# ChangwuLiu/InGVIO

Hardware: AMD Instinct MI355X
Metric: ekf_updates_per_sec (higher is better)
Workload: dtype f64; 1 GPU; BASELINE configs[1]: synthetic stereo MSCKF, 150 feats x 11 clones, state dim N=249 (update at N), 512 independent filters per GPU; step = propagate(k=10)+clone+MSCKF update+marginalise; filters_per_gpu=512, feats=150, clones=11, state_dim=249, imu_steps=10, parallelism=independent filters, 1 rank(s), no data-path collective

## Files before the change

include/ingvio_hip.h:

```cpp
#ifndef INGVIO_HIP_H
#define INGVIO_HIP_H

#include <stddef.h>

#ifdef __cplusplus
extern "C" {
#endif

#define INGVIO_OK 0
#define INGVIO_NO_ROWS 1
#define INGVIO_NEG_DIAG 2
#define INGVIO_REJECTED 3
#define INGVIO_E_ARG (-1)
#define INGVIO_E_CAPACITY (-2)
#define INGVIO_E_HIP (-3)
#define INGVIO_E_NOT_IN_STATE (-4)
#define INGVIO_E_UNSUPPORTED (-5)
#define INGVIO_E_NOT_PD (-6)

typedef struct ingvio_ctx ingvio_ctx;

typedef struct {
    int batch;
    int n_max;
// ... 323 lines not shown
    double psr_noise_amp, dopp_noise_amp;
} ingvio_gnss_epoch_nominal;
int ingvio_gnss_front_stage_nominal(ingvio_ctx* ctx, int b0, int nb, const ingvio_gnss_epoch_nominal* epochs, const ingvio_gnss_opts* opts);
int ingvio_gnss_frame_stage_nominal(ingvio_ctx* ctx, int b0, int nb, const ingvio_gnss_epoch_nominal* epochs, const ingvio_gnss_opts* opts);
int ingvio_debug_gnss_fused_last(ingvio_ctx* ctx);
int ingvio_debug_nominal_update_post(ingvio_ctx* ctx, int b0, int nb, const double* dx, const int* marg_idx);
typedef struct {
    int n_lm;
    const int* lm_var;
    const double* uv;
    const unsigned char* tracked;
} ingvio_landmark_frame_nominal;
int ingvio_landmark_stage_nominal(ingvio_ctx* ctx, int b0, int nb, const ingvio_landmark_frame_nominal* frames,
                                  const ingvio_landmark_opts* opts);
typedef struct {
    int track;
    int anchor;
    double pf[3];
} ingvio_lm_init_cand;
typedef struct {
    int n_cand; const ingvio_lm_init_cand* cand;
    int n_drop; const int* drop_cols;
} ingvio_lm_init_block;
int ingvio_landmark_init_nominal(ingvio_ctx* ctx, int b0, int nb, const ingvio_lm_init_block* blocks, const ingvio_msckf_opts* opts,
                                 double chi2_mult, int do_chi2, int cand_cap,
                                 int* added, int* new_idx, int* slot, double* chi2, double* dx, int* status);
int ingvio_debug_landmark_init_rows(ingvio_ctx* ctx, int b, const ingvio_lm_init_cand* cand, const ingvio_msckf_opts* opts,
                                    int n_drop, const int* drop_cols, double* H_old, double* H_new, double* res, int* m_out);
int ingvio_frame_run(ingvio_ctx* ctx, int restore_prior);
int ingvio_set_frame_parts(ingvio_ctx* ctx, int parts);
int ingvio_set_gram_reduced(ingvio_ctx* ctx, int on);
int ingvio_set_gram_decoupled(ingvio_ctx* ctx, int on);
int ingvio_last_gram_form(ingvio_ctx* ctx);
int ingvio_set_delayed_form(ingvio_ctx* ctx, int mode);
int ingvio_frame_fetch(ingvio_ctx* ctx, int b0, int nb, double* dx_out, int* accepted, int* rows_out);
int ingvio_frame_fetch_begin(ingvio_ctx* ctx, int b0, int nb);
int ingvio_frame_fetch_end(ingvio_ctx* ctx, double* dx_out, int* accepted, int* rows_out);

int ingvio_debug_msckf_info(ingvio_ctx* ctx, int b, double* A_out, int* ncol_out);

int ingvio_debug_info_solution(ingvio_ctx* ctx, int b, double* out, int count);

int ingvio_debug_tracks_read(ingvio_ctx* ctx, int b, unsigned long long* mask, double* uv, double* pf);

int ingvio_debug_staged_frame(ingvio_ctx* ctx, int b, int* n_clones, int* n_feat, int* clone_idx, double* clone_R, double* clone_p,
                              int* anchor, int* dof, unsigned long long* obs_mask, double* pf, double* uv);

int ingvio_debug_read(ingvio_ctx* ctx, long long* out, int n);

int ingvio_profile_enable(ingvio_ctx* ctx, int enable);
int ingvio_profile_select(ingvio_ctx* ctx, const char* kernel_name);
int ingvio_profile_reset(ingvio_ctx* ctx);
int ingvio_profile_get(ingvio_ctx* ctx, const char** names, double* ms, int* calls, int cap);

#ifdef __cplusplus
}
#endif
#endif
```

ingvio_amd/capi.py:

```python
import ctypes as C
import os

import numpy as np

_HERE = os.path.dirname(os.path.abspath(__file__))
LIB_PATH = os.environ.get("INGVIO_HIP_LIB") or os.path.join(_HERE, "lib", "libingvio_hip.so")

c_dp = C.POINTER(C.c_double)
c_ip = C.POINTER(C.c_int)
c_up = C.POINTER(C.c_ulonglong)

OK, NO_ROWS, NEG_DIAG, REJECTED = 0, 1, 2, 3
E_ARG, E_CAPACITY, E_HIP, E_NOT_IN_STATE, E_UNSUPPORTED, E_NOT_PD = -1, -2, -3, -4, -5, -6
R_SCALAR, R_DIAG, R_FULL = 0, 1, 2

EXPORTS = [
    "ingvio_ctx_create", "ingvio_ctx_destroy", "ingvio_sync", "ingvio_ctx_stream", "ingvio_f_max", "ingvio_c_max", "ingvio_last_error", "ingvio_ldp",
    "ingvio_build_id",
    "ingvio_cov_set", "ingvio_cov_get", "ingvio_get_n", "ingvio_cov_get_marginal", "ingvio_cov_snapshot",
    "ingvio_cov_restore", "ingvio_propagate", "ingvio_propagate_fused", "ingvio_augment_clone", "ingvio_marginalize",
    "ingvio_append_independent", "ingvio_ekf_update", "ingvio_chi2_gamma", "ingvio_msckf_update", "ingvio_msckf_update_tri", "ingvio_qr_compress",
    "ingvio_frame_stage", "ingvio_frame_stage_async", "ingvio_frame_set_imu_noise", "ingvio_frame_fetch_begin", "ingvio_frame_fetch_end", "ingvio_tracks_create", "ingvio_frame_stage_tracks", "ingvio_frame_run", "ingvio_set_frame_parts", "ingvio_set_gram_reduced", "ingvio_set_gram_decoupled", "ingvio_last_gram_form", "ingvio_frame_fetch", "ingvio_profile_enable", "ingvio_profile_select",
    "ingvio_profile_reset",
    "ingvio_profile_get", "ingvio_set_msckf_method", "ingvio_set_qr_method", "ingvio_landmark_stage", "ingvio_landmark_run",
    "ingvio_landmark_fetch", "ingvio_frame_run_phase", "ingvio_info_set", "ingvio_debug_read", "ingvio_triangulate",
    "ingvio_gnss_front_stage", "ingvio_gnss_front_fetch", "ingvio_gnss_update_batch", "ingvio_gnss_stage", "ingvio_gnss_run", "ingvio_gnss_fetch", "ingvio_mld", "ingvio_debug_msckf_info", "ingvio_debug_info_solution",
    "ingvio_info_reduce", "ingvio_info_commit", "ingvio_gnss_sat_eval",
    "ingvio_chi2_gamma_multi", "ingvio_ekf_update_batch", "ingvio_add_variable_delayed_invertible", "ingvio_add_variable_delayed", "ingvio_add_variable_delayed_batch", "ingvio_replace_var_linear",
    "ingvio_nominal_create", "ingvio_nominal_set", "ingvio_nominal_get", "ingvio_nominal_box_plus", "ingvio_frame_stage_tracks_nominal",
    "ingvio_nominal_set_gnss", "ingvio_nominal_get_gnss", "ingvio_gnss_front_stage_nominal", "ingvio_landmark_stage_nominal",
    "ingvio_landmark_init_nominal", "ingvio_debug_landmark_init_rows", "ingvio_nominal_tail",
    "ingvio_debug_tracks_read", "ingvio_debug_staged_frame",
    "ingvio_gnss_frame_stage_nominal", "ingvio_debug_gnss_fused_last", "ingvio_debug_nominal_update_post",
    "ingvio_update_stage_tracks_nominal", "ingvio_frame_fetch_tri", "ingvio_set_delayed_form",
    "ingvio_odom_begin", "ingvio_odom_end", "ingvio_cov_get_marginal_batch",
    "ingvio_frame_stage_tracks_nominal_tri", "ingvio_set_first_tri_placement",
]

NOM_NONE, NOM_SE23, NOM_SE3, NOM_VEC3, NOM_SCALAR, NOM_LANDMARK = -1, 0, 1, 2, 3, 4
NOM_VAL = 15
ODOM_COV, ODOM_EUCL, ODOM_DIAG = 1, 2, 4
ODOM_ALL = ODOM_COV | ODOM_EUCL | ODOM_DIAG
ODOM_NONFINITE, ODOM_NEG_DIAG, ODOM_ABSENT = 1, 2, 4
MARGINAL_NS_MAX = 64


class GateBlock(C.Structure):
    _fields_ = [("vidx", C.POINTER(C.c_int)), ("vsize", C.POINTER(C.c_int)), ("k", C.c_int), ("H", C.POINTER(C.c_double)),
                ("ldh", C.c_int), ("m", C.c_int), ("res", C.POINTER(C.c_double))]


class UpdateBlock(C.Structure):
    _fields_ = [("vidx", C.POINTER(C.c_int)), ("vsize", C.POINTER(C.c_int)), ("k", C.c_int), ("H", C.POINTER(C.c_double)),
                ("ldh", C.c_int), ("m", C.c_int), ("res", C.POINTER(C.c_double)), ("R", C.POINTER(C.c_double))]

# ... 1022 lines not shown
        nb = len(steps)
        sa = (FrameStep * nb)(); fa = (MsckfFrame * nb)()
        keeps = []
        for i in range(nb):
            s, k1 = make_step(steps[i]); f, k2 = make_frame(frames[i])
            sa[i] = s; fa[i] = f; keeps.append((k1, k2))
        o, chi2 = make_opts(frames[0], max_accept, compress_rule, selected_variant)
        sg = f64(sigma)

        fn = self.L.ingvio_frame_stage_async if use_async else self.L.ingvio_frame_stage

        def call(_keep=(keeps, chi2, sa, fa, o, sg)):
            self._chk(fn(self.h, b0, nb, sa, fa, C.byref(o), _d(sg), int(enable_gnss), C.c_double(sigma_cb), C.c_double(sigma_rw)))
        return call

    def frame_set_imu_noise(self, b0, noise):
        nz = f64(np.asarray(noise, dtype=np.float64).reshape(-1, 6))
        self._chk(self.L.ingvio_frame_set_imu_noise(self.h, int(b0), nz.shape[0], _d(nz)))

    def frame_run(self, restore_prior=False):
        self._chk(self.L.ingvio_frame_run(self.h, 1 if restore_prior else 0))

    def set_frame_parts(self, parts):
        self._chk(self.L.ingvio_set_frame_parts(self.h, int(parts)))

    def set_gram_reduced(self, on):
        self._chk(self.L.ingvio_set_gram_reduced(self.h, 1 if on else 0))

    def set_gram_decoupled(self, on):
        self._chk(self.L.ingvio_set_gram_decoupled(self.h, 1 if on else 0))

    def last_gram_form(self):
        return int(self.L.ingvio_last_gram_form(self.h))

    def set_delayed_form(self, mode):
        self._chk(self.L.ingvio_set_delayed_form(self.h, int(mode)))

    def frame_fetch(self, b0=0, nb=None):
        nb = self.batch if nb is None else nb
        dx = np.zeros((nb, self.ldp)); acc = np.zeros((nb, self.f_max), dtype=np.int32); rows = np.zeros(nb, dtype=np.int32)
        self._chk(self.L.ingvio_frame_fetch(self.h, b0, nb, _d(dx), _i(acc), _i(rows)))
        return dx, acc, rows

    def frame_fetch_begin(self, b0=0, nb=None):
        nb = self.batch if nb is None else nb
        self._fetch_nb = nb
        self._chk(self.L.ingvio_frame_fetch_begin(self.h, b0, nb))

    def frame_fetch_end(self):
        nb = self._fetch_nb
        dx = np.empty((nb, self.ldp)); acc = np.empty((nb, self.f_max), dtype=np.int32); rows = np.empty(nb, dtype=np.int32)
        self._chk(self.L.ingvio_frame_fetch_end(self.h, _d(dx), _i(acc), _i(rows)))
        return dx, acc, rows

    def triangulate(self, b0, frames, stereo=True, mask_failed=False, **params):
        pr = dict(trans_thres=0.1, huber_epsilon=0.01, conv_precision=5e-7, init_damping=1e-3, outer_loop_max_iter=10,
                  inner_loop_max_iter=10, max_depth=60.0, min_depth=0.2)
        pr.update(params)
        o = TriOpts()
        o.stereo = 1 if stereo else 0
        ref = frames[0] if frames else None
        Rl = f64(ref["R_cl2cr"]).reshape(-1) if ref is not None else np.eye(3).reshape(-1)
        tl = f64(ref["t_cl2cr"]) if ref is not None else np.zeros(3)
        if "R_cl2cr" in params:
            Rl = f64(pr.pop("R_cl2cr")).reshape(-1)
        if "t_cl2cr" in params:
# ... 83 lines not shown
```

ingvio_amd/csrc/capi.hip:

```cpp
#include "../../include/ingvio_hip.h"
#include "dev_common.h"
#include "launch_ekf.h"
#include "launch_msckf.h"
#include "launch_factored.h"
#include "launch_tri.h"
#include "launch_tracks.h"
#include "launch_lm.h"
#include "launch_delayed.h"
#include "launch_qr.h"
#include "launch_chol.h"
#include "launch_gnss.h"
#include "launch_lmbatch.h"
#include "launch_nominal.h"
#include "launch_tail.h"
#include "launch_odom.h"

#include <stdio.h>
#include <stdlib.h>
#include <string.h>
#include <unistd.h>
#include <string>
#include <atomic>
#include <cmath>
#include <condition_variable>
// ... 115 lines not shown
    MsckfOpts st_op;
    std::vector<int> st_gnss;
    std::vector<int> st_marg;
    std::vector<int> st_cidx_hi;
    bool staged;
    double* d_xchg = nullptr;
    bool phase_pending = false;
    struct InputSet {
        double *Phi = nullptr, *G = nullptr, *dt = nullptr, *R = nullptr, *clone_R = nullptr, *clone_p = nullptr, *pf = nullptr, *uv = nullptr,
               *chi2 = nullptr, *noise = nullptr, *prm = nullptr;
        int *gnss = nullptr, *idx = nullptr, *clone_idx = nullptr, *nclones = nullptr, *nfeat = nullptr, *anchor = nullptr, *dof = nullptr;
        unsigned long long* mask = nullptr;
    } alt;
    bool alt_ready = false;
    hipStream_t st2 = nullptr;
    hipEvent_t ev_fork = nullptr, ev_join = nullptr, ev_ref = nullptr;
    hipEvent_t ev_fetch = nullptr;
    int fetch_b0 = 0, fetch_nb = 0;
    hipStream_t st_copy = nullptr;
    hipEvent_t ev_copy = nullptr, ev_free[2] = { nullptr, nullptr };
    bool copy_pending = false, free_valid[2] = { false, false };
    int set_id = 0;
    struct PinSlab { char* p = nullptr; size_t cap = 0; hipEvent_t ev = nullptr; bool busy = false; };
    PinSlab pin[4];
    int pin_next = 0;
    struct PartStream { hipStream_t st = nullptr; hipEvent_t ev_gate = nullptr, ev_apply = nullptr, ev_done = nullptr; };
    PartStream part[4];
    int parts_alloc = 0;
    int parts_req = -1;
    int gram_reduced = 1;
    int delayed_form = 0;
    int gram_decoupled = 1;
    int gram_form_last = 0;
    int gram_red_last = 0;
    bool split_pending = false;
    hipEvent_t tok_last = nullptr;
    hipEvent_t ev_split_fork = nullptr;
    hipStream_t run_st = nullptr;
    hipEvent_t tok_wait = nullptr, tok_rec = nullptr;
    struct Tracks { double *uv = nullptr, *pf = nullptr; unsigned long long* mask = nullptr; int t_max = 0; char* stage[2] = { nullptr, nullptr }; size_t stage_cap = 0; } trk;
    struct Nominal {
        int vmax = 0, ir = 0, dr = 0;
        int* ih = nullptr; double* dv = nullptr;
        int* ih_snap = nullptr; double* dv_snap = nullptr;
        double* dx = nullptr;
        std::vector<int> h_ih, h_ih_snap;
        bool has_snap = false;
        bool pending = false;
        bool frame = false;
        hipEvent_t ev = nullptr; bool ev_valid = false;
        bool noprop = false, tri_on = false, tri_ran = false;
        int tri_fmx = 0;
        bool tri_fetched = false; int tri_b0 = 0, tri_nb = 0;
        ingvio_tri_opts tri;
        int* d_tri_track = nullptr;
        int tri_place = 0;
        bool tri_staged = false;
        int* d_tri_ok_st = nullptr; double* d_tri_pf_st = nullptr;
    } nom;
    struct TailWs { char *in = nullptr, *ws = nullptr, *h_out = nullptr; size_t in_cap = 0, ws_cap = 0, out_cap = 0; } tl;
    struct OdomOut {
        double *d = nullptr, *h = nullptr; hipEvent_t ev = nullptr; bool pending = false; int b0 = 0, nb = 0;
        int *cols = nullptr, *ns = nullptr; double* blk = nullptr; size_t cols_cap = 0, blk_cap = 0;
    } od;
    bool prof;
    std::vector<ProfRec> recs;
// ... 606 lines not shown
                if (used) c->recs.push_back({ PF_GATE2, L.prof_a, L.prof_b });
                else { hipEventDestroy(L.prof_a); hipEventDestroy(L.prof_b); }
                L.prof_a = nullptr; L.prof_b = nullptr; L.prof_used = nullptr;
            }
            if (grc) return INGVIO_E_UNSUPPORTED;
        }
        c->gram_red_last = 0; c->gram_form_last = 0;
        L.gram_red = frame_step && phase == 0 && c->gram_reduced; L.gram_was_red = &c->gram_red_last;
        L.gram_dec = c->gram_decoupled; L.gram_form = &c->gram_form_last;
        { ProfScope p(c, PF_GRAM); L.stage = 1; launch_factored(L, c->run_st); }
        L.gram_was_red = nullptr; L.gram_form = nullptr;
        if (c->tok_rec) HIPCHK(c, hipEventRecord(c->tok_rec, c->run_st));
    }
    if (forked) {
        HIPCHK(c, hipStreamWaitEvent(c->st2, c->ev_fork, 0));
        L.stage = 6; launch_factored(L, c->st2);
        HIPCHK(c, hipEventRecord(c->ev_ref, c->st2));
        L.stage = 7; launch_factored(L, c->st2);
        HIPCHK(c, hipEventRecord(c->ev_join, c->st2));
    }
    if (phase == 1) return last_launch(c);
    if (forked) {
        ProfScope p(c, PF_INFO);
        HIPCHK(c, hipStreamWaitEvent(c->run_st, c->ev_ref, 0));
        L.stage = 8; launch_factored(L, c->run_st);
        HIPCHK(c, hipStreamWaitEvent(c->run_st, c->ev_join, 0));
        L.stage = 9; launch_factored(L, c->run_st);
    } else {
        if (big) { ProfScope p(c, PF_INFO); L.stage = 5; launch_factored(L, c->run_st); }
        { ProfScope p(c, PF_INFO); L.stage = 2; launch_factored(L, c->run_st); }
    }
    if (gnss_fuse) { if (int rc = gnss_in_frame_launch(c, b0, nb, L)) return rc; }
    if (phase == 2 && c->tok_wait) HIPCHK(c, hipStreamWaitEvent(c->run_st, c->tok_wait, 0));
    { ProfScope p(c, PF_APPLY); L.stage = 3; launch_factored(L, c->run_st); }
    if (phase == 2 && c->tok_rec) HIPCHK(c, hipEventRecord(c->tok_rec, c->run_st));
    return last_launch(c);
}

int run_msckf(ingvio_ctx* c, int b0, int nb, const MsckfOpts& op, int stereo, int fmax_used)
{
    if (c->method == 1) return run_msckf_factored(c, b0, nb, op, stereo, fmax_used);
    c->gram_red_last = 0; c->gram_form_last = 0;
    MsckfLaunch L;
    memset(&L, 0, sizeof L);
    L.stereo = stereo; L.cv = view(c); L.fv = fview(c); L.op = op; L.b0 = b0; L.nb = nb;
    L.fmax_used = fmax_used > 0 ? fmax_used : 1;
    L.gamma = c->d_gamma; L.accept = c->d_accept; L.used = c->d_used;
    L.Rpart = c->d_Rpart + (size_t)b0 * c->G * c->rstride; L.chunk_used = c->d_chunk_used + (size_t)b0 * c->G;
    L.G = c->G; L.rstride = c->rstride;
    L.Hout = c->d_H + (size_t)b0 * c->hstride; L.res_out = c->d_res + (size_t)b0 * c->mld;
    L.colmap = c->d_colmap + (size_t)b0 * c->cstride; L.m_out = c->d_m + b0; L.nc_out = c->d_nc + b0;
    L.mld = c->mld; L.hstride = c->hstride; L.cstride = c->cstride;
    { ProfScope p(c, PF_GATE); L.stage = 0; if (launch_msckf(L, c->st)) return INGVIO_E_UNSUPPORTED; }
    { ProfScope p(c, PF_FOLD); L.stage = 1; launch_msckf(L, c->st); }
    { ProfScope p(c, PF_MERGE); L.stage = 2; launch_msckf(L, c->st); }
    EkfLaunch E;
    memset(&E, 0, sizeof E);
    E.cv = view(c); E.b0 = b0; E.nb = nb; E.H = L.Hout; E.res = L.res_out; E.colmap = L.colmap; E.m = L.m_out; E.nc = L.nc_out;
    E.noise = c->d_noise + b0; E.r_kind = 0; E.mld = c->mld; E.hstride = c->hstride; E.cstride = c->cstride; E.nstride = 1;
    E.Y = c->d_Y + (size_t)b0 * c->ystride; E.ystride = c->ystride; E.dx = c->d_dx; E.status = c->d_status;
    E.m_cap = 6 * c->d.c_max; E.nc_cap = 6 * c->d.c_max;
    { ProfScope p(c, PF_EKF_CORE); launch_ekf_core(E, c->st); }
    { ProfScope p(c, PF_DOWNDATE); launch_downdate(E, c->d.n_max, c->st); }
    return last_launch(c);
}

// ... 111 lines not shown
        c->nom.frame = plan != nullptr;
        c->nom.noprop = upd; c->nom.tri_on = false; c->nom.tri_staged = false;
        c->st_stereo = opts->stereo; c->st_enable_gnss = enable_gnss;
        if (!c->staged || fmx > c->st_fmax_used) c->st_fmax_used = fmx;
        c->staged = true;
        return INGVIO_OK;
    }
};

}

extern "C" {

int ingvio_ctx_create(const ingvio_ctx_desc* desc, ingvio_ctx** out)
{
    if (!desc || !out || desc->batch < 1 || desc->n_max < 21 || desc->c_max < 1 || desc->f_max < 1) return INGVIO_E_ARG;
    if (desc->c_max > bigwin_cmax()) return INGVIO_E_CAPACITY;
    if (desc->m_max > 128) return INGVIO_E_CAPACITY;
    int ndev = 0;
    if (hipGetDeviceCount(&ndev) != hipSuccess || ndev <= desc->device) return INGVIO_E_HIP;
    ingvio_ctx* c = new ingvio_ctx();
    c->d = *desc;
    if (c->d.m_max < 1) c->d.m_max = 32;
    c->err.clear();
    if (hipSetDevice(desc->device) != hipSuccess) { delete c; return INGVIO_E_HIP; }
    c->own_stream = desc->stream == nullptr;
    if (c->own_stream) {
        if (hipStreamCreateWithFlags(&c->st, hipStreamNonBlocking) != hipSuccess) { delete c; return INGVIO_E_HIP; }
    } else c->st = (hipStream_t)desc->stream;
    c->run_st = c->st;
    if (const char* e = getenv("INGVIO_FRAME_PARTS")) c->parts_req = atoi(e);
    if (const char* e = getenv("INGVIO_GRAM_REDUCED")) c->gram_reduced = atoi(e) != 0;
    if (const char* e = getenv("INGVIO_GRAM_DECOUPLED")) c->gram_decoupled = atoi(e) != 0;
    if (desc->c_max > 16) {
        int lo = 0, hi = 0;
        hipDeviceGetStreamPriorityRange(&lo, &hi);
        if (hipStreamCreateWithPriority(&c->st2, hipStreamNonBlocking, hi) != hipSuccess) c->st2 = nullptr;
        if (c->st2 && (hipEventCreateWithFlags(&c->ev_fork, hipEventDisableTiming) != hipSuccess ||
                       hipEventCreateWithFlags(&c->ev_ref, hipEventDisableTiming) != hipSuccess ||
                       hipEventCreateWithFlags(&c->ev_join, hipEventDisableTiming) != hipSuccess)) { hipStreamDestroy(c->st2); c->st2 = nullptr; }
    }
    const int B = desc->batch;
    c->ldp = (desc->n_max + 15) & ~15;
    const int cls0 = desc->c_max > 16 ? bigwin_cmax() : msckf_cmax_class(desc->c_max);
    const int cpad = cls0 > desc->c_max ? cls0 : desc->c_max;
    const int mcap = c->d.m_max > 6 * cpad ? c->d.m_max : 6 * cpad;
    c->mld = (mcap + 15) & ~15;
    c->nc_cap = c->ldp > mcap ? c->ldp : mcap;
    c->G = (desc->c_max > 16 ? 256 : 512) / B;
    { const int gmax = desc->c_max > 16 ? 32 : 16; if (c->G > gmax) c->G = gmax; }
    if (c->G < 1) c->G = 1;
#ifdef INGVIO_ALT_KERNELS
    if (const char* e = getenv("INGVIO_GRAM_CHUNKS")) { const int g = atoi(e); if (g >= 1 && g <= 64) c->G = g; }
#endif
    c->cls = msckf_cmax_class(desc->c_max);
    const int ncm = 6 * desc->c_max;
    c->rstride = ncm * (ncm + 1);
    c->hstride = c->mld * c->nc_cap;
    c->cstride = c->nc_cap;
    c->ystride = std::max(c->ldp * (c->mld + 4), c->mld * (c->mld + 1));
    c->has_snap = false; c->staged = false; c->prof = false;
    c->method = 1;
#ifdef INGVIO_ALT_KERNELS
    if (const char* e = getenv("INGVIO_MSCKF_METHOD")) c->method = (!strcmp(e, "dense") || !strcmp(e, "0")) ? 0 : 1;
#endif
    memset(c->prof_ms, 0, sizeof c->prof_ms); memset(c->prof_calls, 0, sizeof c->prof_calls);
// ... 3264 lines not shown
    const bool gnss_fuse = gnss_folds(c);
    if (P > 1 && c->method == 1 && !lm_in_frame(c) && c->d.c_max <= 16 && (!gnss_in_frame(c) || gnss_fuse) && B >= 16 * P)
        return frame_run_split(c, restore_prior, P, gnss_fuse);
    return frame_run_whole(c, restore_prior);
}

int ingvio_frame_run(ingvio_ctx* c, int restore_prior) { return frame_run_impl(c, restore_prior, 0); }
int ingvio_set_frame_parts(ingvio_ctx* c, int parts)
{
    if (!c || parts < -1 || parts > 4) return INGVIO_E_ARG;
    ENTER(c);
    c->parts_req = parts == 0 ? 1 : parts;
    return INGVIO_OK;
}
int ingvio_set_gram_reduced(ingvio_ctx* c, int on)
{
    if (!c) return INGVIO_E_ARG;
    ENTER(c);
    c->gram_reduced = on ? 1 : 0;
    return INGVIO_OK;
}
int ingvio_set_gram_decoupled(ingvio_ctx* c, int on)
{
    if (!c) return INGVIO_E_ARG;
    ENTER(c);
    c->gram_decoupled = on ? 1 : 0;
    return INGVIO_OK;
}
int ingvio_last_gram_form(ingvio_ctx* c)
{
    if (!c) return INGVIO_E_ARG;
    return c->gram_form_last;
}
int ingvio_set_delayed_form(ingvio_ctx* c, int mode)
{
    if (!c) return INGVIO_E_ARG;
    ENTER(c);
    if (mode < 0 || mode > 2) { c->err = "ingvio_set_delayed_form: mode is 0, 1 or 2"; return INGVIO_E_ARG; }
    if (phase_busy(c)) return INGVIO_E_ARG;
    if (c->nom.pending) { c->err = "ingvio_set_delayed_form: a frame staged from the device nominal state has not run yet"; return INGVIO_E_ARG; }
    c->delayed_form = mode;
    return INGVIO_OK;
}
int ingvio_frame_run_phase(ingvio_ctx* c, int restore_prior, int phase)
{
    if (phase < 0 || phase > 2) return INGVIO_E_ARG;
    return frame_run_impl(c, restore_prior, phase);
}

int ingvio_info_set(ingvio_ctx* c, int b, const double* A, int ncol, int n_accepted)
{
    ENTER(c);
    if (check_range(c, b, 1) || !A || ncol < 6 || (size_t)ncol * (ncol + 1) > (size_t)c->rstride || n_accepted < 0) return INGVIO_E_ARG;
    std::vector<int> used(c->G, 0);
    used[0] = n_accepted;
    int rc = up(c, c->d_Rpart + (size_t)b * c->G * c->rstride, A, 8 * (size_t)ncol * (ncol + 1));
    rc |= up(c, c->d_chunk_used + (size_t)b * c->G, used.data(), sizeof(int) * (size_t)c->G);
    if (rc) return INGVIO_E_HIP;
    HIPCHK(c, hipStreamSynchronize(c->st));
    return INGVIO_OK;
}

namespace {
__global__ __launch_bounds__(256) void k_info_reduce(const double* __restrict__ Apart, const int* __restrict__ chunk_used, int G, int rstride,
                                                     int cnt, double* __restrict__ out)
{
// ... 277 lines not shown
```

ingvio_amd/csrc/kernels_factored.hip:

```cpp
#include <algorithm>
#include <stdlib.h>
#include <string.h>
#include "launch_factored.h"

#include "gate_kernel.h"
#include "gate5_kernel.h"
#include "gate5m_kernel.h"

#define GATE_FPW 1
template <int CMAX, bool STEREO>
__global__ __launch_bounds__(GATE_FPW * WAVE) __attribute__((amdgpu_waves_per_eu(2, 4))) void k_feat_gate3(
    CovView cv, FrameView fv, MsckfOpts op, int b0, int nb, int fmax_used, double* __restrict__ gamma_out,
    int* __restrict__ accept_out, double* __restrict__ rec_out)
{
    gate3_body<CMAX, STEREO, GATE_FPW, false>(cv, fv, op, b0, nb, fmax_used, gamma_out, accept_out, rec_out);
}

#ifndef GATE4_WPE
#define GATE4_WPE 2
#endif
#ifndef GATE4_WPE_MAX
#define GATE4_WPE_MAX 6
#endif
template <int CMAX>
// ... 964 lines not shown
                if (YW > 0 && updY) {
#pragma unroll
                    for (int k4 = 0; k4 < KY; ++k4) acc = __builtin_amdgcn_mfma_f64_16x16x4f64(yfrag[1][k4], bfy[k4], acc, 0, 0, 0);
                }
                store_tile(tiR[1], tj, acc, pv[1][q]);
            }
        }
        if (tjj == 4 * TW) dbg_stamp(45);
        if (more) stage_store(buf ^ 1, stg_out);
        if (tjj == 4 * TW) dbg_stamp(46);
#pragma unroll
        for (int d = 0; d < PF; ++d)
#pragma unroll
            for (int h = 0; h < 2; ++h)
#pragma unroll
                for (int q = 0; q < TW; ++q)
#pragma unroll
                    for (int r = 0; r < 4; ++r) pq[d][h][q][r] = pq[d + 1][h][q][r];
#if defined(APPLY_ABL) && (APPLY_ABL & 8)
        __builtin_amdgcn_wave_barrier();
#else
        lds_barrier();
#endif
        if (tjj == 4 * TW) dbg_stamp(47);
    };
    for (int tjj = 0; tjj <= tjmax; tjj += 2 * TW) {
        sweep_step(tjj, 0, stgA, stgB);
        if (tjj + TW <= tjmax) sweep_step(tjj + TW, 1, stgB, stgA);
    }
    if ((upd || updY) && __any(neg_diag) && lane == 0) atomicOr(&status[b], 2);
    dbg_stamp(13);
}

template <int NC>
__global__ __launch_bounds__(256) void k_apply_T_flat(CovView cv, int b0, const double* __restrict__ Mall, int mstride, const double* __restrict__ Pcall,
                                                      int ystride, const int* __restrict__ m_all, const int* __restrict__ marg_idx, int msize,
                                                      const int* __restrict__ pc_base, double* __restrict__ Tall, size_t tstride,
                                                      double* __restrict__ dx_all)
{
    constexpr int MP = (NC + 3) & ~3, K4 = MP / 4, JT = (MP + 15) / 16;
    const int bl = blockIdx.y, b = b0 + bl;
    if (m_all[bl] == 0) return;
    const int n = cv.n[b], ld = cv.ldp, nt = (n + 15) >> 4;
    const int wave = threadIdx.x >> 6, lane = threadIdx.x & 63, l15 = lane & 15, kq = lane >> 4;
    const int t = blockIdx.x * 4 + wave;
    if (t >= nt * JT) return;
    const int ti = t / JT, tj = t - ti * JT;
    const double* P = cov_ptr(cv, b);
    const int pcb = pc_base[bl];
    const double* Pc = pcb >= 0 ? P + (size_t)pcb * ld : Pcall + (size_t)bl * ystride;
    const double* M = Mall + (size_t)bl * mstride;
    const double* tvec = M + (size_t)MP * MP;
    const int ra = min(16 * ti + l15, n - 1), jc = min(16 * tj + l15, MP - 1);
    double pf[K4], mf[K4];
#pragma unroll
    for (int k4 = 0; k4 < K4; ++k4) pf[k4] = (Pc + (size_t)(4 * k4) * ld)[ra + kq * ld];
#pragma unroll
    for (int k4 = 0; k4 < K4; ++k4) mf[k4] = (M + (size_t)(4 * k4) * MP)[kq * MP + jc];
    const int midx = marg_idx ? marg_idx[bl] : -1;
    if (tj == 0) {
        double d = 0.0;
#pragma unroll
        for (int k4 = 0; k4 < K4; ++k4) d += pf[k4] * tvec[4 * k4 + kq];
        d += __shfl_xor(d, 16, WAVE);
        d += __shfl_xor(d, 32, WAVE);
        const bool marg_row = midx >= 0 && ra >= midx && ra < midx + msize;
// ... 274 lines not shown
    }
    if (blockIdx.x == 0 && threadIdx.x == 0) used_out[bl] = total;
}

int factored_rec_size(int cmax)
{
    if (cmax > 16) return cmax <= bigwin_cmax() ? bigwin_rec_size() : 0;
    const int cls = cmax <= 6 ? 6 : (cmax <= 11 ? 11 : (cmax <= 12 ? 12 : 16));
    return rec_size(cls);
}

int launch_factored(const FactoredLaunch& L, hipStream_t st)
{
    if (L.fv.cmax > 16) return launch_bigwin(L, st);
    const int cm_sel = (L.c_used > 0 && L.c_used <= L.fv.cmax) ? L.c_used : L.fv.cmax;
    const int ncm = 6 * cm_sel;
    if (L.stage == 10) {
        const int MP = ncm <= 36 ? 36 : (ncm <= 66 ? 68 : (ncm <= 72 ? 72 : 96));
        hipLaunchKernelGGL(k_info_dx, dim3((L.n_cap + 255) / 256, L.nb), dim3(256), 0, st, L.cv, L.b0, MP, L.T, L.mstride, L.Pc, L.ystride, L.m_out,
                           L.pc_base, L.marg_idx, L.marg_size, L.dx);
        return 0;
    }
    if (L.stage == 4) {
        const int nt = (L.n_cap + 15) / 16;
#define POSTCOLS_DISPATCH(NC)                                                                                           \
        hipLaunchKernelGGL((k_post_cols<NC>), dim3((nt + 3) / 4, L.nb), dim3(256), 0, st, L.cv, L.b0, L.T, L.mstride, L.Pc, L.ystride, L.m_out, \
                           L.pc_base, L.gcolmap, L.gnc, L.gcstride, L.gW, L.gWstride);
        if (ncm <= 36) { POSTCOLS_DISPATCH(36) } else if (ncm <= 66) { POSTCOLS_DISPATCH(66) } else if (ncm <= 72) { POSTCOLS_DISPATCH(72) } else { POSTCOLS_DISPATCH(96) }
#undef POSTCOLS_DISPATCH
        return 0;
    }
    if (L.stage == 3) {
        const int nt = (L.n_cap + 15) / 16, wgpf = ((nt + 1) / 2 + 3) / 4, nb8 = (L.nb + 7) / 8 * 8;
#ifdef INGVIO_ALT_KERNELS
        static const bool tw1 = [] { const char* e = getenv("INGVIO_APPLY_TW"); return !(e && e[0] == '2'); }();
#define APPLY_TW2(NC) else if (!tw1) hipLaunchKernelGGL((k_info_apply<NC, 2>), dim3(nb8 * wgpf), dim3(256), 0, st, L.cv, L.b0, L.nb, wgpf, L.T, L.mstride, L.Pc, \
                           L.ystride, L.m_out, L.dx, L.status, L.marg_idx, L.marg_size, L.pc_base);
#else
#define APPLY_TW2(NC)
#endif
        if (!L.gY && L.Tflat && L.nb <= L.flat_nb) {
            const int JTx = ncm <= 36 ? 3 : (ncm <= 72 ? 5 : 6);
#define FLAT_DISPATCH(NC)                                                                                             \
            hipLaunchKernelGGL((k_apply_T_flat<NC>), dim3((nt * JTx + 3) / 4, L.nb), dim3(256), 0, st, L.cv, L.b0, L.T, L.mstride, L.Pc, L.ystride, \
                               L.m_out, L.marg_idx, L.marg_size, L.pc_base, L.Tflat, L.tfstride, L.dx);                 \
            hipLaunchKernelGGL((k_apply_sym_flat<NC>), dim3((nt * (nt + 1) / 2 + 3) / 4, L.nb), dim3(256), 0, st, L.cv, L.b0, L.Pc, L.ystride, \
                               L.m_out, L.marg_idx, L.marg_size, L.pc_base, L.Tflat, L.tfstride, L.status);
            if (ncm <= 36) { FLAT_DISPATCH(36) } else if (ncm <= 66) { FLAT_DISPATCH(66) } else if (ncm <= 72) { FLAT_DISPATCH(72) } else { FLAT_DISPATCH(96) }
#undef FLAT_DISPATCH
            return 0;
        }
#define APPLY_DISPATCH(NC)                                                                                            \
        if (L.gY) { hipLaunchKernelGGL((k_info_apply<NC, 1, 16>), dim3(nb8 * wgpf), dim3(256), 0, st, L.cv, L.b0, L.nb, wgpf, L.T, L.mstride, L.Pc, \
                           L.ystride, L.m_out, L.dx, L.status, L.marg_idx, L.marg_size, L.pc_base, L.gY, L.gYstride, L.gm, flip); if (flip) *L.did_flip = 1; } \
        APPLY_TW2(NC)                                                                                                 \
        else { hipLaunchKernelGGL((k_info_apply<NC, 1>), dim3(nb8 * wgpf), dim3(256), 0, st, L.cv, L.b0, L.nb, wgpf, L.T, L.mstride, L.Pc, \
                           L.ystride, L.m_out, L.dx, L.status, L.marg_idx, L.marg_size, L.pc_base, (const double*)nullptr, (size_t)0, (const int*)nullptr, flip); if (flip) *L.did_flip = 1; }
        int* const flip = (L.marg_idx && L.did_flip) ? L.flip_cnt : nullptr;
        if (ncm <= 36) { APPLY_DISPATCH(36) } else if (ncm <= 66) { APPLY_DISPATCH(66) } else if (ncm <= 72) { APPLY_DISPATCH(72) } else { APPLY_DISPATCH(96) }
#undef APPLY_DISPATCH
#undef APPLY_TW2
        return 0;
    }
    if (L.stage == 2 && L.G > 1 && L.Asum) {
        hipLaunchKernelGGL(k_chunk_sum, dim3((L.rstride + 255) / 256, L.nb), dim3(256), 0, st, L.Apart, L.chunk_used, L.G, L.rstride, L.Asum, L.used_sum);
        FactoredLaunch L1 = L;
        L1.Apart = L.Asum; L1.chunk_used = L.used_sum; L1.G = 1; L1.Asum = nullptr;
        return launch_factored(L1, st);
    }
    if (L.stage == 2) {
#ifdef INGVIO_ALT_KERNELS
        static const bool use_gj = [] { const char* e = getenv("INGVIO_INFO_SOLVE"); return e && !strcmp(e, "gj"); }();
#else
        constexpr bool use_gj = false;
#endif
        if (!use_gj && launch_info_solve(L, st) == 0) return 0;
#define INFO_DISPATCH(NC)                                                                                                   \
        {                                                                                                                   \
            const size_t sm = sizeof(double) * (size_t)NC * (2 * NC + 1) + sizeof(int) * (size_t)NC + 16;                     \
            hipFuncSetAttribute((const void*)k_info_update<NC>, hipFuncAttributeMaxDynamicSharedMemorySize, (int)sm);         \
            hipLaunchKernelGGL(k_info_update<NC>, dim3(L.nb), dim3(INFO_NT), sm, st, L.cv, L.fv, L.b0, L.Apart, L.chunk_used, \
                               L.G, L.rstride, L.noise, L.T, L.mstride, L.Pc, L.ystride, L.dx, L.m_out, L.nc_out, L.status,  \
                               L.marg_idx, L.pc_base);                                                                      \
        }
        if (ncm <= 36) { INFO_DISPATCH(36) } else if (ncm <= 66) { INFO_DISPATCH(66) } else if (ncm <= 72) { INFO_DISPATCH(72) } else { INFO_DISPATCH(96) }
#undef INFO_DISPATCH
        return 0;
    }
    const int cm = cm_sel;
    const int cls = cm <= 6 ? 6 : (cm <= 11 ? 11 : (cm <= 12 ? 12 : (cm <= 16 ? 16 : -1)));
    if (cls < 0) return -1;
// ... 21 lines not shown
```

ingvio_amd/csrc/launch_factored.h:

```cpp
#pragma once
#include "dev_common.h"

#ifndef INGVIO_APPLY_FLAT_NB
#define INGVIO_APPLY_FLAT_NB 64
#endif
constexpr int APPLY_FLAT_NB = INGVIO_APPLY_FLAT_NB;

struct FactoredLaunch {
    int stage;
    int stereo;
    CovView cv;
    FrameView fv;
    MsckfOpts op;
    int b0, nb, fmax_used;
    double* gamma;
    int* accept;
    int* used;
    double* rec;
    double* Apart;
    double* Asum;
    int* used_sum;
    double* Tflat;
    size_t tfstride;
    int flat_nb;
    int* chunk_used;
    int G, rstride;
    const double* noise;
    double* T;
    int mstride, n_cap;
    double* Pc;
    int ystride;
    double* dx;
    int* m_out;
    int* nc_out;
    int* status;
    const int* marg_idx;
    int marg_size;
    int* pc_base;
    int* flip_cnt;
    int* did_flip;
    int gram_red;
    int* gram_was_red;
    int gram_dec;
    int* gram_form;
    double* big_sg;
    double* big_wk;
    int ncol_cap;
    int c_used;
    const int* gcolmap;
    const int* gnc;
    int gcstride;
    double* gW;
    size_t gWstride;
    const double* gY;
    size_t gYstride;
    const int* gm;
    hipEvent_t prof_a, prof_b;
    int* prof_used;
};
#include <hip/hip_ext.h>
#define LAUNCH_GATE(L, kernel, grid, block, shmem, st, ...)                                                             \
    do {                                                                                                                \
        if ((L).prof_a) { hipExtLaunchKernelGGL(kernel, grid, block, shmem, st, (L).prof_a, (L).prof_b, 0, __VA_ARGS__); if ((L).prof_used) *(L).prof_used = 1; } \
        else hipLaunchKernelGGL(kernel, grid, block, shmem, st, __VA_ARGS__);                                           \
    } while (0)

int launch_factored(const FactoredLaunch& L, hipStream_t st);
int launch_info_solve(const FactoredLaunch& L, hipStream_t st);
int dbg_read_solve(long long* out, int n);
int factored_rec_size(int cmax);
int dbg_read_factored(long long* out, int n);

int launch_bigwin(const FactoredLaunch& L, hipStream_t st);
void launch_apply64(const FactoredLaunch& L, hipStream_t st, int mp, double* T, size_t tstride, int ldt);
size_t bigwin_sg_doubles(int G);
size_t bigwin_wk_doubles();
int bigwin_rec_size();
// ... 3 lines not shown
```

Baseline: 1.103 million updates/s.

## Add resident one-block-per-filter info-apply kernel with LDS-staged Pc and MFMA

Adds a new covariance-apply kernel that runs one 512-thread workgroup per filter. It keeps the Pc rows in LDS, computes T = M·Pc once per row-tile with f64 MFMA, and then sweeps lower-triangle tile pairs with prefetched P loads, writing both triangles through an LDS transpose. It replaces the multi-workgroup-per-filter apply, with the aim of avoiding recomputation and redundant global Pc and M reads across workgroups. The new path is on by default for frame steps when the sizes fit, and can be switched off by an env var or a new API call. The cost is heavy LDS use and lower occupancy: one large block per filter.

```diff
diff --git a/include/ingvio_hip.h b/include/ingvio_hip.h
--- a/include/ingvio_hip.h
+++ b/include/ingvio_hip.h
@@ -379,6 +379,8 @@
 int ingvio_set_gram_reduced(ingvio_ctx* ctx, int on);
 int ingvio_set_gram_decoupled(ingvio_ctx* ctx, int on);
 int ingvio_last_gram_form(ingvio_ctx* ctx);
+int ingvio_set_apply_resident(ingvio_ctx* ctx, int on);
+int ingvio_last_apply_form(ingvio_ctx* ctx);
 int ingvio_set_delayed_form(ingvio_ctx* ctx, int mode);
 int ingvio_frame_fetch(ingvio_ctx* ctx, int b0, int nb, double* dx_out, int* accepted, int* rows_out);
 int ingvio_frame_fetch_begin(ingvio_ctx* ctx, int b0, int nb);
diff --git a/ingvio_amd/capi.py b/ingvio_amd/capi.py
--- a/ingvio_amd/capi.py
+++ b/ingvio_amd/capi.py
@@ -20,7 +20,7 @@
     "ingvio_cov_set", "ingvio_cov_get", "ingvio_get_n", "ingvio_cov_get_marginal", "ingvio_cov_snapshot",
     "ingvio_cov_restore", "ingvio_propagate", "ingvio_propagate_fused", "ingvio_augment_clone", "ingvio_marginalize",
     "ingvio_append_independent", "ingvio_ekf_update", "ingvio_chi2_gamma", "ingvio_msckf_update", "ingvio_msckf_update_tri", "ingvio_qr_compress",
-    "ingvio_frame_stage", "ingvio_frame_stage_async", "ingvio_frame_set_imu_noise", "ingvio_frame_fetch_begin", "ingvio_frame_fetch_end", "ingvio_tracks_create", "ingvio_frame_stage_tracks", "ingvio_frame_run", "ingvio_set_frame_parts", "ingvio_set_gram_reduced", "ingvio_set_gram_decoupled", "ingvio_last_gram_form", "ingvio_frame_fetch", "ingvio_profile_enable", "ingvio_profile_select",
+    "ingvio_frame_stage", "ingvio_frame_stage_async", "ingvio_frame_set_imu_noise", "ingvio_frame_fetch_begin", "ingvio_frame_fetch_end", "ingvio_tracks_create", "ingvio_frame_stage_tracks", "ingvio_frame_run", "ingvio_set_frame_parts", "ingvio_set_gram_reduced", "ingvio_set_gram_decoupled", "ingvio_last_gram_form", "ingvio_set_apply_resident", "ingvio_last_apply_form", "ingvio_frame_fetch", "ingvio_profile_enable", "ingvio_profile_select",
     "ingvio_profile_reset",
     "ingvio_profile_get", "ingvio_set_msckf_method", "ingvio_set_qr_method", "ingvio_landmark_stage", "ingvio_landmark_run",
     "ingvio_landmark_fetch", "ingvio_frame_run_phase", "ingvio_info_set", "ingvio_debug_read", "ingvio_triangulate",
@@ -1109,6 +1109,12 @@
 
     def last_gram_form(self):
         return int(self.L.ingvio_last_gram_form(self.h))
+
+    def set_apply_resident(self, on):
+        self._chk(self.L.ingvio_set_apply_resident(self.h, 1 if on else 0))
+
+    def last_apply_form(self):
+        return int(self.L.ingvio_last_apply_form(self.h))
 
     def set_delayed_form(self, mode):
         self._chk(self.L.ingvio_set_delayed_form(self.h, int(mode)))
diff --git a/ingvio_amd/csrc/capi.hip b/ingvio_amd/csrc/capi.hip
--- a/ingvio_amd/csrc/capi.hip
+++ b/ingvio_amd/csrc/capi.hip
@@ -171,6 +171,8 @@
     int delayed_form = 0;
     int gram_decoupled = 1;
     int gram_form_last = 0;
+    int apply_resident = 1;
+    int apply_form_last = 0;
     int gram_red_last = 0;
     bool split_pending = false;
     hipEvent_t tok_last = nullptr;
@@ -843,6 +845,8 @@
     }
     if (gnss_fuse) { if (int rc = gnss_in_frame_launch(c, b0, nb, L)) return rc; }
     if (phase == 2 && c->tok_wait) HIPCHK(c, hipStreamWaitEvent(c->run_st, c->tok_wait, 0));
+    c->apply_form_last = 0;
+    L.apply_res = frame_step && phase == 0 && c->apply_resident; L.apply_form = &c->apply_form_last;
     { ProfScope p(c, PF_APPLY); L.stage = 3; launch_factored(L, c->run_st); }
     if (phase == 2 && c->tok_rec) HIPCHK(c, hipEventRecord(c->tok_rec, c->run_st));
     return last_launch(c);
@@ -1020,6 +1024,7 @@
     if (const char* e = getenv("INGVIO_FRAME_PARTS")) c->parts_req = atoi(e);
     if (const char* e = getenv("INGVIO_GRAM_REDUCED")) c->gram_reduced = atoi(e) != 0;
     if (const char* e = getenv("INGVIO_GRAM_DECOUPLED")) c->gram_decoupled = atoi(e) != 0;
+    if (const char* e = getenv("INGVIO_APPLY_RESIDENT")) c->apply_resident = atoi(e) != 0;
     if (desc->c_max > 16) {
         int lo = 0, hi = 0;
         hipDeviceGetStreamPriorityRange(&lo, &hi);
@@ -4350,6 +4355,18 @@
     if (!c) return INGVIO_E_ARG;
     return c->gram_form_last;
 }
+int ingvio_set_apply_resident(ingvio_ctx* c, int on)
+{
+    if (!c) return INGVIO_E_ARG;
+    ENTER(c);
+    c->apply_resident = on ? 1 : 0;
+    return INGVIO_OK;
+}
+int ingvio_last_apply_form(ingvio_ctx* c)
+{
+    if (!c) return INGVIO_E_ARG;
+    return c->apply_form_last;
+}
 int ingvio_set_delayed_form(ingvio_ctx* c, int mode)
 {
     if (!c) return INGVIO_E_ARG;
diff --git a/ingvio_amd/csrc/kernels_factored.hip b/ingvio_amd/csrc/kernels_factored.hip
--- a/ingvio_amd/csrc/kernels_factored.hip
+++ b/ingvio_amd/csrc/kernels_factored.hip
@@ -1020,6 +1020,222 @@
     dbg_stamp(13);
 }
 
+#ifndef APPLY_RES_PF
+#define APPLY_RES_PF 2
+#endif
+constexpr int APPLY_RES_ROWS = 256, APPLY_RES_NW = 8;
+#ifndef APPLY_RES_ABL
+#define APPLY_RES_ABL 0
+#endif
+#if APPLY_RES_ABL & 4
+#define APPLY_RES_MFMA(a, b, c) double4_f{ fma((a), (b), (c)[0]), (c)[1], (c)[2], (c)[3] }
+#else
+#define APPLY_RES_MFMA(a, b, c) __builtin_amdgcn_mfma_f64_16x16x4f64((a), (b), (c), 0, 0, 0)
+#endif
+template <int NC>
+constexpr size_t apply_res_lds_bytes() { return sizeof(double) * ((size_t)APPLY_RES_ROWS * (((NC + 3) & ~3) + 2) + APPLY_RES_NW * 16 * 17); }
+
+template <int NC>
+__global__ __launch_bounds__(64 * APPLY_RES_NW) void k_info_apply_res(CovView cv, int b0, const double* __restrict__ Mall, int mstride,
+                                                                      const double* __restrict__ Pcall, int ystride, const int* __restrict__ m_all,
+                                                                      double* __restrict__ dx_all, int* __restrict__ status,
+                                                                      const int* __restrict__ marg_idx, int msize, const int* __restrict__ pc_base)
+{
+    constexpr int MP = (NC + 3) & ~3, K4 = MP / 4, JT = (MP + 15) / 16, LS = MP + 2, PF = APPLY_RES_PF;
+    extern __shared__ __attribute__((aligned(16))) char smem_raw[];
+    double* sPc = reinterpret_cast<double*>(smem_raw);
+    double (*sV)[16][17] = reinterpret_cast<double (*)[16][17]>(sPc + (size_t)APPLY_RES_ROWS * LS);
+    const int bl = blockIdx.x, b = b0 + bl;
+    const bool upd = m_all[bl] != 0;
+    const int midx = marg_idx[bl];
+    const bool fused = midx >= 0;
+    if (!upd && !fused) return;
+    const int n = cv.n[b], ld = cv.ldp;
+    const int no = fused ? n - msize : n, nt = (no + 15) >> 4;
+    if (nt > APPLY_RES_ROWS / 16) return;
+    const int tid = threadIdx.x, wave = __builtin_amdgcn_readfirstlane(tid >> 6), lane = tid & 63;
+    const int rowL = nt - 1 - wave, rowS = wave;
+    const bool onL = 2 * wave < nt, onS = wave < rowL;
+    const double* P = cov_ptr(cv, b);
+    double* dst = fused ? cov_alt_ptr(cv, b) : cov_ptr(cv, b);
+    const int pcb = upd ? pc_base[bl] : -1;
+    const double* Pc = pcb >= 0 ? P + (size_t)pcb * ld : Pcall + (size_t)bl * ystride;
+    const double* M = Mall + (size_t)bl * mstride;
+    const double* tvec = M + (size_t)MP * MP;
+    const int l15 = lane & 15, kq = lane >> 4;
+    auto src_of = [&](int o) __attribute__((always_inline)) { return (fused && o >= midx) ? o + msize : o; };
+
+    bool neg_diag = false;
+    auto store_tile = [&](int ti, int tj, const double4_f& acc, const double (&pv)[4]) __attribute__((always_inline)) {
+        const int col = tj * 16 + l15, row0 = ti * 16 + kq, row2 = ti * 16 + l15, col20 = tj * 16 + kq;
+        double v[4], t[4];
+#pragma unroll
+        for (int r = 0; r < 4; ++r) { v[r] = pv[r] - acc[r]; sV[wave][kq + 4 * r][l15] = v[r]; }
+        __builtin_amdgcn_wave_barrier();
+#pragma unroll
+        for (int r = 0; r < 4; ++r) t[r] = sV[wave][l15][kq + 4 * r];
+        __builtin_amdgcn_wave_barrier();
+        double* d1 = dst + col + (size_t)row0 * ld;
+        double* d2 = dst + row2 + (size_t)col20 * ld;
+#if APPLY_RES_ABL & 1
+        if (v[0] + v[1] + v[2] + v[3] + t[0] + t[1] + t[2] + t[3] == 1.2345e-300) dst[0] = v[0];
+        else if (ti < 0)
+#endif
+        if (ti > tj && ti * 16 + 15 < no) {
+#pragma unroll
+            for (int r = 0; r < 4; ++r) APPLY_STORE(d1 + (size_t)(4 * r) * ld, v[r]);
+#pragma unroll
+            for (int r = 0; r < 4; ++r) APPLY_STORE(d2 + (size_t)(4 * r) * ld, t[r]);
+        } else if (ti > tj) {
+#pragma unroll
+            for (int r = 0; r < 4; ++r) if (row0 + 4 * r < no) APPLY_STORE(d1 + (size_t)(4 * r) * ld, v[r]);
+            if (row2 < no) {
+#pragma unroll
+                for (int r = 0; r < 4; ++r) APPLY_STORE(d2 + (size_t)(4 * r) * ld, t[r]);
+            }
+        } else {
+#pragma unroll
+            for (int r = 0; r < 4; ++r) {
+                const int row = row0 + 4 * r;
+                if (row < no && col < no && row >= col) APPLY_STORE(d1 + (size_t)(4 * r) * ld, v[r]);
+                neg_diag |= row == col && row < no && v[r] < 0.0;
+            }
+#pragma unroll
+            for (int r = 0; r < 4; ++r) {
+                const int col2 = col20 + 4 * r;
+                if (row2 < no && col2 < no && row2 > col2) APPLY_STORE(d2 + (size_t)(4 * r) * ld, t[r]);
+            }
+        }
+    };
+    auto load_p = [&](int ti, int tj, double (&pv)[4]) __attribute__((always_inline)) {
+        const int col = tj * 16 + l15, row0 = ti * 16 + kq;
+#if APPLY_RES_ABL & 2
+#pragma unroll
+        for (int r = 0; r < 4; ++r) pv[r] = 1.0 + r;
+        if (ti < 0)
+#endif
+        if (ti > tj && ti * 16 + 15 < no) {
+            const double* p0 = P + src_of(col);
+#pragma unroll
+            for (int r = 0; r < 4; ++r) pv[r] = APPLY_LOADP(p0 + (size_t)src_of(row0 + 4 * r) * ld);
+        } else if (ti > tj) {
+            const double* p0 = P + src_of(col);
+#pragma unroll
+            for (int r = 0; r < 4; ++r) pv[r] = APPLY_LOADP(p0 + (size_t)src_of(min(row0 + 4 * r, no - 1)) * ld);
+        } else {
+#pragma unroll
+            for (int r = 0; r < 4; ++r) {
+                const int row = row0 + 4 * r;
+                pv[r] = (row < no && col < no && row >= col) ? APPLY_LOADP(&P[src_of(col) + (size_t)src_of(row) * ld]) : 0.0;
+            }
+        }
+    };
+    double pq[PF + 1][2][4];
+    auto load_step = [&](int tj, double (&d)[2][4]) __attribute__((always_inline)) {
+        if (onL && tj <= rowL) load_p(rowL, tj, d[0]);
+        if (onS && tj <= rowS) load_p(rowS, tj, d[1]);
+    };
+
+    double pcf[2][K4], tf[2][K4];
+#pragma unroll
+    for (int h = 0; h < 2; ++h)
+#pragma unroll
+        for (int k4 = 0; k4 < K4; ++k4) { pcf[h][k4] = 0.0; tf[h][k4] = 0.0; }
+    if (upd) {
+#pragma unroll
+        for (int h = 0; h < 2; ++h)
+            if (h == 0 ? onL : onS) {
+                const int ti = h == 0 ? rowL : rowS;
+                const int ra = src_of(min(ti * 16 + l15, no - 1));
+#pragma unroll
+                for (int k4 = 0; k4 < K4; ++k4) pcf[h][k4] = (Pc + (size_t)(4 * k4) * ld)[ra + kq * ld];
+            }
+    }
+    if (upd && fused && wave == 0) {
+        for (int q = lane; q < msize; q += WAVE) {
+            double d = 0.0;
+            for (int k = 0; k < MP; ++k) d += Pc[midx + q + (size_t)k * ld] * tvec[k];
+            dx_all[(size_t)b * ld + midx + q] = d;
+        }
+    }
+    if (upd && onL) {
+        double mf[2][K4];
+        auto load_m = [&](int jt, double (&m)[K4]) __attribute__((always_inline)) {
+            const int jc = min(jt * 16 + l15, MP - 1);
+#pragma unroll
+            for (int k4 = 0; k4 < K4; ++k4) m[k4] = (M + (size_t)(4 * k4) * MP)[kq * MP + jc];
+        };
+        load_m(0, mf[0]);
+#pragma unroll
+        for (int h = 0; h < 2; ++h)
+            if (h == 0 || onS) {
+                const int ti = h == 0 ? rowL : rowS;
+                const int ra = src_of(min(ti * 16 + l15, no - 1));
+#pragma unroll
+                for (int k4 = 0; k4 < K4; ++k4) sPc[(size_t)(ti * 16 + l15) * LS + 4 * k4 + kq] = pcf[h][k4];
+                double d = 0.0;
+#pragma unroll
+                for (int k4 = 0; k4 < K4; ++k4) d += pcf[h][k4] * tvec[4 * k4 + kq];
+                d += __shfl_xor(d, 16, WAVE);
+                d += __shfl_xor(d, 32, WAVE);
+                if (kq == 0 && ti * 16 + l15 < no) dx_all[(size_t)b * ld + ra] = d;
+            }
+#pragma unroll
+        for (int jt = 0; jt < JT; ++jt) {
+            if (jt + 1 < JT) load_m(jt + 1, mf[(jt + 1) & 1]);
+#pragma unroll
+            for (int h = 0; h < 2; ++h)
+                if (h == 0 || onS) {
+                    double4_f acc = { 0.0, 0.0, 0.0, 0.0 };
+#pragma unroll
+                    for (int k4 = 0; k4 < K4; ++k4) acc = __builtin_amdgcn_mfma_f64_16x16x4f64(mf[jt & 1][k4], pcf[h][k4], acc, 0, 0, 0);
+#pragma unroll
+                    for (int r = 0; r < 4; ++r) if (4 * jt + r < K4) tf[h][4 * jt + r] = acc[r];
+                }
+        }
+    }
+#pragma unroll
+    for (int d = 0; d < PF; ++d) load_step(d, pq[d]);
+    __syncthreads();
+    if (fused && tid == 0) { cv.cur[b] ^= 1; cv.n[b] = n - msize; }
+
+    if (onL) {
+#pragma unroll 1
+        for (int tj = 0; tj <= rowL; ++tj) {
+            load_step(tj + PF, pq[PF]);
+            const bool doS = onS && tj <= rowS;
+            double bfrag[K4];
+            if (upd) {
+#pragma unroll
+                for (int k4 = 0; k4 < K4; ++k4) bfrag[k4] = sPc[(size_t)(16 * tj + l15) * LS + 4 * k4 + kq];
+            }
+            if (doS) {
+                double4_f acc = { 0.0, 0.0, 0.0, 0.0 };
+                if (upd) {
+#pragma unroll
+                    for (int k4 = 0; k4 < K4; ++k4) acc = APPLY_RES_MFMA(tf[1][k4], bfrag[k4], acc);
+                }
+                store_tile(rowS, tj, acc, pq[0][1]);
+            }
+            {
+                double4_f acc = { 0.0, 0.0, 0.0, 0.0 };
+                if (upd) {
+#pragma unroll
+                    for (int k4 = 0; k4 < K4; ++k4) acc = APPLY_RES_MFMA(tf[0][k4], bfrag[k4], acc);
+                }
+                store_tile(rowL, tj, acc, pq[0][0]);
+            }
+#pragma unroll
+            for (int d = 0; d < PF; ++d)
+#pragma unroll
+                for (int h = 0; h < 2; ++h)
+#pragma unroll
+                    for (int r = 0; r < 4; ++r) pq[d][h][r] = pq[d + 1][h][r];
+        }
+    }
+    if (upd && __any(neg_diag) && lane == 0) atomicOr(&status[b], 2);
+}
+
 template <int NC>
 __global__ __launch_bounds__(256) void k_apply_T_flat(CovView cv, int b0, const double* __restrict__ Mall, int mstride, const double* __restrict__ Pcall,
                                                       int ystride, const int* __restrict__ m_all, const int* __restrict__ marg_idx, int msize,
@@ -1360,6 +1576,7 @@
     }
     if (L.stage == 3) {
         const int nt = (L.n_cap + 15) / 16, wgpf = ((nt + 1) / 2 + 3) / 4, nb8 = (L.nb + 7) / 8 * 8;
+        if (L.apply_form) *L.apply_form = 0;
 #ifdef INGVIO_ALT_KERNELS
         static const bool tw1 = [] { const char* e = getenv("INGVIO_APPLY_TW"); return !(e && e[0] == '2'); }();
 #define APPLY_TW2(NC) else if (!tw1) hipLaunchKernelGGL((k_info_apply<NC, 2>), dim3(nb8 * wgpf), dim3(256), 0, st, L.cv, L.b0, L.nb, wgpf, L.T, L.mstride, L.Pc, \
@@ -1385,6 +1602,23 @@
         else { hipLaunchKernelGGL((k_info_apply<NC, 1>), dim3(nb8 * wgpf), dim3(256), 0, st, L.cv, L.b0, L.nb, wgpf, L.T, L.mstride, L.Pc, \
                            L.ystride, L.m_out, L.dx, L.status, L.marg_idx, L.marg_size, L.pc_base, (const double*)nullptr, (size_t)0, (const int*)nullptr, flip); if (flip) *L.did_flip = 1; }
         int* const flip = (L.marg_idx && L.did_flip) ? L.flip_cnt : nullptr;
+        if (L.apply_res && flip && !L.gY && L.nb > APPLY_FLAT_NB && L.cv.ldp <= APPLY_RES_ROWS && L.n_cap <= APPLY_RES_ROWS && ncm <= 66) {
+#define APPLY_RES_DISPATCH(NC)                                                                                        \
+            {                                                                                                         \
+                static bool attr_set = false;                                                                         \
+                if (!attr_set) {                                                                                      \
+                    hipFuncSetAttribute((const void*)k_info_apply_res<NC>, hipFuncAttributeMaxDynamicSharedMemorySize, (int)apply_res_lds_bytes<NC>()); \
+                    attr_set = true;                                                                                  \
+                }                                                                                                     \
+                hipLaunchKernelGGL((k_info_apply_res<NC>), dim3(L.nb), dim3(64 * APPLY_RES_NW), apply_res_lds_bytes<NC>(), st, L.cv, L.b0, L.T,  \
+                                   L.mstride, L.Pc, L.ystride, L.m_out, L.dx, L.status, L.marg_idx, L.marg_size, L.pc_base);  \
+            }
+            if (ncm <= 36) APPLY_RES_DISPATCH(36) else APPLY_RES_DISPATCH(66)
+#undef APPLY_RES_DISPATCH
+            *L.did_flip = 1;
+            if (L.apply_form) *L.apply_form = 1;
+            return 0;
+        }
         if (ncm <= 36) { APPLY_DISPATCH(36) } else if (ncm <= 66) { APPLY_DISPATCH(66) } else if (ncm <= 72) { APPLY_DISPATCH(72) } else { APPLY_DISPATCH(96) }
 #undef APPLY_DISPATCH
 #undef APPLY_TW2
diff --git a/ingvio_amd/csrc/launch_factored.h b/ingvio_amd/csrc/launch_factored.h
--- a/ingvio_amd/csrc/launch_factored.h
+++ b/ingvio_amd/csrc/launch_factored.h
@@ -43,6 +43,8 @@
     int* gram_was_red;
     int gram_dec;
     int* gram_form;
+    int apply_res;
+    int* apply_form;
     double* big_sg;
     double* big_wk;
     int ncol_cap;
```

Measured after the change: 1.115 million updates/s (median of 6 runs). 1.1% higher.
